# sinamalakouti/CDDMSL

Hardware: AMD Instinct MI355X
Metric: images/sec (train step) VOC+Clipart RN50-C4 (higher is better)
Workload: dtype bf16

## Files before the change

### cddmsl_amd/csrc/gemm_conv.hip

```cpp
#include "common.h"
#include <cstdlib>
#include <type_traits>

namespace {

constexpr int BM = 128, BN = 128, KCH = 8;

struct FastDiv {
  unsigned mul, shr, d;
};
static inline FastDiv make_fastdiv(unsigned d) {
  FastDiv f;
  f.d = d;
  unsigned s = 0;
  while ((1ull << s) < d) ++s;
  f.shr = s;
  f.mul = (unsigned)(((1ull << 32) * ((1ull << s) - d)) / d + 1);
  return f;
}
__device__ __forceinline__ unsigned fdiv(unsigned n, const FastDiv& f) { return (__umulhi(n, f.mul) + n) >> f.shr; }

template <typename T> __device__ __forceinline__ float affine(float v, float sc, float bi) {
  return sizeof(T) <= 2 ? __builtin_fmaf(v, sc, bi) : v * sc + bi;
}
// ... 1821 lines not shown
      continue;
    }
    const unsigned vy = (unsigned)(((tile * 32 + 4 * hh) * p.ldy + r) * ES), vmk = (unsigned)(((tile * 32 + 4 * hh) * p.ldm + r) * ES);
#pragma unroll
    for (int nt = 0; nt < NT; ++nt)
#pragma unroll
      for (int g = 0; g < 16; ++g) {
        const int row = (g & 3) + 8 * (g >> 2);
        float v = affine<T>(acc[nt][g], sc[nt], bi[nt]);
        asm("v_max_f32 %0, %1, %2" : "=v"(v) : "v"(v), "s"(relu_floor));
        if (p.relu_mask) {
          float mv;
          if (ES == 2) mv = bf2f((unsigned)__builtin_amdgcn_raw_buffer_load_b16(rm, vmk, (row * p.ldm + nt * 32) * ES, 0));
          else mv = __builtin_bit_cast(float, __builtin_amdgcn_raw_buffer_load_b32(rm, vmk, (row * p.ldm + nt * 32) * ES, 0));
          if (!(mv > 0.f)) v = 0.f;
        }
        if (ES == 2) __builtin_amdgcn_raw_buffer_store_b16((unsigned short)f2bf(v), ry, vy, (row * p.ldy + nt * 32) * ES, 0);
        else __builtin_amdgcn_raw_buffer_store_b32(__builtin_bit_cast(unsigned, v), ry, vy, (row * p.ldy + nt * 32) * ES, 0);
      }
  }
}

static thread_local int g_last_kernel = 0;
static thread_local int g_plan_only = 0;
static thread_local int g_batch = 1;
static inline int g_batch_peek() { return g_batch; }

__device__ __forceinline__ void blds16(__amdgpu_buffer_rsrc_t r, unsigned voff, unsigned soff, void* l) {
  __builtin_amdgcn_raw_ptr_buffer_load_lds(r, (__attribute__((address_space(3))) void*)l, 16, (int)voff, (int)soff, 0, 0);
}

template <typename T, bool RPOOL, int EPI, bool PRE = false>
__device__ __forceinline__ void tile_epilogue(const ConvArgs& p, f32x16 (&acc)[4][2], float* ep, int wr, int wc, int lane, int m0, int n0,
                                              const u32x4 (*pre)[4] = nullptr, const f32x4* sb = nullptr) {
  constexpr int ES = Mma<T>::ES;
  const int r32 = lane & 31, hh = lane >> 5;
  const int cg = lane & 7, rr = lane >> 3;
  const int n = n0 + wc * 64 + cg * 8;
  float sc[8], bi[8];
#pragma unroll
  for (int j = 0; j < 8; ++j) {
    if (sb) { sc[j] = sb[j >> 2][j & 3]; bi[j] = sb[2 + (j >> 2)][j & 3]; }
    else { sc[j] = p.scale ? p.scale[n + j] : 1.f; bi[j] = p.bias ? p.bias[n + j] : 0.f; }
  }
  const bool has_res = EPI < 0 ? p.residual != nullptr : (EPI & 1) != 0;
  const bool has_msk = EPI < 0 ? p.relu_mask != nullptr : (EPI & 2) != 0;
  const bool f32out = EPI < 0 && (ES == 4 || p.out_f32 != 0);
  const int eso = f32out ? 4 : 2;
  const float relu_floor = p.relu ? 0.f : -__builtin_inff();
  const long rows = p.M - m0;
  auto mk = [&](const char* base, long ld, int es) {
    long bytes = rows * ld * es;
    if (bytes > 0x7fffffffL) bytes = 0x7fffffffL;
    return __builtin_amdgcn_make_buffer_rsrc((void*)(base + (long)m0 * ld * es), 0, base ? (int)bytes : 0, 0x00020000);
  };
// ... 31 lines not shown
        else if (has_res && !rf32) rres_[i][q] = __builtin_amdgcn_raw_buffer_load_b128(rres, vr, (a * 32 + 8 * i) * p.ldr * ES + q * 16, CDDMSL_LOAD_AUX);
        if (has_msk) rmsk_[i][q] = __builtin_amdgcn_raw_buffer_load_b128(rmsk, vm, (a * 32 + 8 * i) * p.ldm * ES + q * 16, CDDMSL_LOAD_AUX);
      }
  };
  if (PRE && DEPTH == 2) {
#pragma unroll
    for (int d = 0; d < 2; ++d)
#pragma unroll
      for (int i = 0; i < 4; ++i) {
        if (EPI & 1) {
          rresb[d % DEPTH][i][0] = pre[d][i];
          if (EPI & 2) rmskb[d % DEPTH][i][0] = __builtin_amdgcn_raw_buffer_load_b128(rmsk, vm, (d * 32 + 8 * i) * p.ldm * ES, CDDMSL_LOAD_AUX);
        } else rmskb[d % DEPTH][i][0] = pre[d][i];
      }
  } else if (DEPTH == 2 && !rf32) { fetch(0, rresb[0], rmskb[0]); fetch(1, rresb[DEPTH - 1], rmskb[DEPTH - 1]); }
  auto put = [&](auto A) {
    constexpr int a = decltype(A)::value;
#pragma unroll
    for (int b = 0; b < 2; ++b)
#pragma unroll
      for (int g = 0; g < 16; ++g)
        *(float*)(wbase[(b << 2) ^ (g & 3)] + ((g & 3) + 8 * (g >> 2)) * 256 + (a & 1) * 8192) = acc[a][b][g];
  };
  auto pass = [&](auto A) {
    constexpr int a = decltype(A)::value;
    if (DEPTH == 1) fetch(a, rresb[0], rmskb[0]);
    if (rf32) {
#pragma unroll
      for (int f = 0; f < 8; ++f)
        rresb[(f >> 2) % DEPTH][f & 3][0] = __builtin_amdgcn_raw_buffer_load_b128(rres, vr, (a * 32 + 8 * (f >> 1)) * p.ldr * 4 + (f & 1) * 16, 0);
    }
    u32x4 (*rres_)[ES / 2] = rresb[a % DEPTH];
    u32x4 (*rmsk_)[ES / 2] = rmskb[a % DEPTH];
    asm volatile("s_waitcnt lgkmcnt(0)" ::: "memory");
    f32x4 val[4][2];
#pragma unroll
    for (int i = 0; i < 4; ++i) {
      const int row = rr + 8 * i;
      const f32x4* src = (const f32x4*)(ep + (a & 1) * 2048 + row * 64 + ((cg ^ (row & 7)) << 3));
      val[i][0] = src[0]; val[i][1] = src[1];
    }
    asm volatile("" ::: "memory");
    if constexpr (a + 1 < 4) put(std::integral_constant<int, a + 1>{});
    asm volatile("" ::: "memory");
#pragma unroll
    for (int i = 0; i < 4; ++i) {
      const f32x4 v0 = val[i][0], v1 = val[i][1];
      float v[8] = {v0[0], v0[1], v0[2], v0[3], v1[0], v1[1], v1[2], v1[3]};
#pragma unroll
      for (int j = 0; j < 8; ++j) v[j] = affine<T>(v[j], sc[j], bi[j]);
      if (rf32) {
#pragma unroll
        for (int j = 0; j < 4; ++j) {
          v[j] += __builtin_bit_cast(f32x4, rresb[((2 * i) >> 2) % DEPTH][(2 * i) & 3][0])[j];
          v[4 + j] += __builtin_bit_cast(f32x4, rresb[((2 * i + 1) >> 2) % DEPTH][(2 * i + 1) & 3][0])[j];
        }
      } else if (RPOOL) {
        if (ES == 2) {
#pragma unroll
          for (int j = 0; j < 4; ++j) { v[2 * j] += 0.25f * bf2f(rres_[i][0][j] & 0xffff); v[2 * j + 1] += 0.25f * bf2f(rres_[i][0][j] >> 16); }
        } else {
#pragma unroll
          for (int j = 0; j < 4; ++j) {
            v[j] += 0.25f * __builtin_bit_cast(f32x4, rres_[i][0])[j]; v[4 + j] += 0.25f * __builtin_bit_cast(f32x4, rres_[i][ES / 2 - 1])[j];
          }
        }
      } else if (has_res) {
        if (ES == 2) {
#pragma unroll
// ... 19 lines not shown
          }
        }
#pragma unroll
        for (int j = 0; j < 8; ++j) if (!(mv[j] > 0.f)) v[j] = 0.f;
      }
      const unsigned so = (unsigned)((a * 32 + 8 * i) * p.ldy * eso);
      if (emit8) {
#pragma unroll
        for (int j = 0; j < 8; ++j) am8 = absmax_bits(am8, v[j]);
        const u32x2 o8 = {pack4_e4m3(v[0] * q8s, v[1] * q8s, v[2] * q8s, v[3] * q8s), pack4_e4m3(v[4] * q8s, v[5] * q8s, v[6] * q8s, v[7] * q8s)};
        __builtin_amdgcn_raw_buffer_store_b64(o8, ry8, vy8, (unsigned)((a * 32 + 8 * i) * p.ldy), CDDMSL_STORE_AUX);
        asm volatile("s_nop 4" ::: "memory");
        asm volatile("" :: "v"(o8));
      }
      if (f32out) {
        const u32x4 o0 = {__builtin_bit_cast(unsigned, v[0]), __builtin_bit_cast(unsigned, v[1]), __builtin_bit_cast(unsigned, v[2]), __builtin_bit_cast(unsigned, v[3])};
        const u32x4 o1 = {__builtin_bit_cast(unsigned, v[4]), __builtin_bit_cast(unsigned, v[5]), __builtin_bit_cast(unsigned, v[6]), __builtin_bit_cast(unsigned, v[7])};
        __builtin_amdgcn_raw_buffer_store_b128(o0, ry, vy, so, CDDMSL_STORE_AUX);
        __builtin_amdgcn_raw_buffer_store_b128(o1, ry, vy, so + 16, CDDMSL_STORE_AUX);
        asm volatile("s_nop 4" ::: "memory");
        asm volatile("" :: "v"(o0), "v"(o1));
      } else {
        const u32x4 o = {pack2bf(v[0], v[1]), pack2bf(v[2], v[3]), pack2bf(v[4], v[5]), pack2bf(v[6], v[7])};
        if (p.nt_out) __builtin_amdgcn_raw_buffer_store_b128(o, ry, vy, so, CDDMSL_STORE_AUX);
        else __builtin_amdgcn_raw_buffer_store_b128(o, ry, vy, so, 0);
        asm volatile("s_nop 4" ::: "memory");
        asm volatile("" :: "v"(o));
      }
    }
    if (DEPTH == 2 && a + 2 < 4 && !rf32) fetch(a + 2, rresb[a % DEPTH], rmskb[a % DEPTH]);
  };
  put(std::integral_constant<int, 0>{});
  pass(std::integral_constant<int, 0>{});
  pass(std::integral_constant<int, 1>{});
  pass(std::integral_constant<int, 2>{});
  pass(std::integral_constant<int, 3>{});
  if (emit8 && p.amax8) {
    am8 = wave_max_u(am8);
    if (lane == 0) atomicMax(p.amax8 + (blockIdx.x & 63), am8);
  }
}

template <typename T, bool TAPS, bool RPOOL = false, int EPI = -1, bool PERSIST = false, bool SPLITK = false>
__global__ __launch_bounds__(512) void k_conv_fwd256(ConvArgs p) {
  __shared__ __attribute__((aligned(16))) u32x4 lds[2 * 2 * 2 * 128 * KCH];
  const int t_in = threadIdx.x;
  p.x += (long)blockIdx.y * p.bx; p.w += (long)blockIdx.y * p.bw; p.y += (long)blockIdx.y * p.by;
  const int ntn = p.Cout >> 8;
  const int ntiles = PERSIST ? (p.tile_limit ? p.tile_limit : ntn * ((p.M + 255) >> 8)) : 0;
  int lbid = PERSIST ? (int)((blockIdx.x & 7) * (gridDim.x >> 3) + (blockIdx.x >> 3))
           : SPLITK ? p.tile0 + (int)(blockIdx.x / (unsigned)p.ksplits) : xcd_remap(blockIdx.x, gridDim.x);
  const int kt0 = SPLITK ? (int)(blockIdx.x % (unsigned)p.ksplits) * p.kper : 0;
  if (PERSIST && lbid >= ntiles) return;
  for (;;) {
  int t = t_in;
  if (PERSIST) asm volatile("" : "+v"(t));
  const int lane = t & 63;
#ifdef CDDMSL_TILE_STAMPS
  const unsigned long long ts_entry = __builtin_amdgcn_s_memrealtime();
#endif
  const int wvu = __builtin_amdgcn_readfirstlane(t >> 6);
  const int wr = wvu >> 2, wc = wvu & 3;
  const int tile_n = lbid % ntn, tile_m = lbid / ntn;
  const int m0 = tile_m * 256, n0 = tile_n * 256;
  const int cl = (t & 7) ^ ((t >> 4) & 7);
  const int nkt = SPLITK ? min(p.kper, (p.Kc >> 3) - kt0) : (p.Kc >> 3);
  const int tpt = p.cpp >> 3;

  auto rowoff = [&](int m, int& iy0, int& ix0) {
    const unsigned tq = fdiv((unsigned)m, p.dWo), ox = m - tq * p.Wo;
    const unsigned img = fdiv(tq, p.dHo), oy = tq - img * p.Ho;
    iy0 = (int)oy * p.stride - p.pad; ix0 = (int)ox * p.stride - p.pad;
    return (((long)img * p.Hi + iy0) * p.Wi + ix0) * p.xrs * 16;
  };
  int iyb, ixb;
  const long base_a = rowoff(m0, iyb, ixb);
  const __amdgpu_buffer_rsrc_t ra_rsrc = __builtin_amdgcn_make_buffer_rsrc((void*)(p.x + base_a), 0, 0x7fffffff, 0x00020000);
  const __amdgpu_buffer_rsrc_t rb_rsrc = __builtin_amdgcn_make_buffer_rsrc((void*)(p.w + (long)n0 * p.wrs * 16), 0, 0x7fffffff, 0x00020000);
  unsigned va[2][2], vinv[2][2], vb[2][2];
  int iy0[2][2], ix0[2][2];
#pragma unroll
  for (int h = 0; h < 2; ++h)
#pragma unroll
    for (int i = 0; i < 2; ++i) {
      const int m = m0 + i * 128 + h * 64 + (t >> 3);
      const bool vm = m < p.M;
      const long ro = rowoff(vm ? m : m0, iy0[h][i], ix0[h][i]);
      va[h][i] = (unsigned)(ro - base_a) + cl * 16;
      if (!vm) { iy0[h][i] = -(1 << 20); if (!TAPS) va[h][i] |= 0x80000000u; }
      vinv[h][i] = 0;
      vb[h][i] = (unsigned)(((2 * i + (t >> 8)) * 64 + h * 32 + ((t >> 3) & 31)) * p.wrs + cl) * 16;
    }
  if (TAPS) {
    unsigned xm[2][2] = {{0, 0}, {0, 0}};
    for (int kx = 0; kx < p.KW; ++kx)
#pragma unroll
      for (int h = 0; h < 2; ++h)
#pragma unroll
        for (int i = 0; i < 2; ++i) xm[h][i] |= ((unsigned)(ix0[h][i] + kx) >= (unsigned)p.Wi ? 1u : 0u) << kx;
    const unsigned full = (1u << p.KW) - 1u;
    for (int ky = 0; ky < p.KH; ++ky)
#pragma unroll
      for (int h = 0; h < 2; ++h)
#pragma unroll
        for (int i = 0; i < 2; ++i) vinv[h][i] |= ((unsigned)(iy0[h][i] + ky) >= (unsigned)p.Hi ? full : xm[h][i]) << (ky * p.KW);
  }
  const int step_col = (p.xrs - (p.cpp - KCH)) * 16;
  const int step_row = ((p.Wi - (p.KW - 1)) * p.xrs - (p.cpp - KCH)) * 16;
  int left[2] = {tpt, tpt}, tap[2] = {0, 0}, kxs[2] = {0, 0};
  unsigned soa[2] = {0, 0}, sob[2] = {0, 0};
  if (SPLITK) {
    const int tap0 = TAPS ? kt0 / tpt : 0, within = TAPS ? kt0 - tap0 * tpt : kt0;
    const int ky0 = TAPS ? tap0 / p.KW : 0, kx0 = tap0 - ky0 * p.KW;
#pragma unroll
    for (int h = 0; h < 2; ++h) {
      left[h] = tpt - (TAPS ? within : 0); tap[h] = tap0; kxs[h] = kx0;
      soa[h] = (unsigned)((ky0 * p.Wi + kx0) * p.xrs * 16 + within * KCH * 16);
      sob[h] = (unsigned)(kt0 * KCH * 16);
    }
  }

  char* const L = (char*)lds;
  auto stageA = [&](auto H, int buf) {
    constexpr int h = decltype(H)::value;
    char* dst = L + (buf << 16) + (h << 14) + wvu * 1024;
#pragma unroll
    for (int i = 0; i < 2; ++i) {
      unsigned v = va[h][i];
      if (TAPS) v |= __builtin_amdgcn_ubfe(vinv[h][i], (unsigned)tap[h], 1u) << 31;
      blds16(ra_rsrc, v, soa[h], dst + i * 8192);
    }
    if (TAPS) {
      int step = KCH * 16;
      if (--left[h] == 0) {
        left[h] = tpt; ++tap[h];
        if (++kxs[h] == p.KW) { kxs[h] = 0; step = step_row; } else step = step_col;
      }
      soa[h] += step;
    } else soa[h] += KCH * 16;
  };
  auto stageB = [&](auto J, int buf) {
    constexpr int j = decltype(J)::value;
    char* dst = L + (buf << 16) + (1 << 15) + (j << 14) + wvu * 1024;
#pragma unroll
    for (int i = 0; i < 2; ++i) blds16(rb_rsrc, vb[j][i], sob[j], dst + i * 8192);
    sob[j] += KCH * 16;
  };
  using I0 = std::integral_constant<int, 0>;
  using I1 = std::integral_constant<int, 1>;

  f32x16 acc[4][2];
#pragma unroll
  for (int a = 0; a < 4; ++a)
#pragma unroll
    for (int b = 0; b < 2; ++b)
#pragma unroll
      for (int r = 0; r < 16; ++r) acc[a][b][r] = 0.f;

  const int r32 = lane & 31, hh = lane >> 5, sw = (r32 >> 1) & 7;
  unsigned ada[4], adb[4];
#pragma unroll
  for (int ks = 0; ks < 4; ++ks) {
    ada[ks] = (unsigned)(((wr * 64 + r32) * KCH + ((2 * ks + hh) ^ sw)) * 16);
    adb[ks] = (unsigned)(((wc * 32 + r32) * KCH + ((2 * ks + hh) ^ sw)) * 16 + (1 << 15));
  }
  u32x4 fa0[2][4], fa1[2][4], fb0[4], fb1[4];
  auto readA = [&](auto I, u32x4 (*fa)[4]) {
    constexpr int i = decltype(I)::value;
// ... 20 lines not shown
  unsigned long long st_sum[4] = {0, 0, 0, 0}, st_last = 0;
#define CDDMSL_STAMP(K) { asm volatile("s_waitcnt lgkmcnt(0)" ::: "memory"); unsigned long long tt_ = __builtin_readcyclecounter(); \
                          asm volatile("s_waitcnt lgkmcnt(0)" ::: "memory"); st_sum[K] += tt_ - st_last; st_last = tt_; }
#else
#define CDDMSL_STAMP(K)
#endif
#define CDDMSL_PHASE_SYNC_IN()                                                      \
  CDDMSL_STAMP(0)                                                                   \
  __builtin_amdgcn_sched_barrier(0);                                                \
  __builtin_amdgcn_s_barrier();                                                     \
  asm volatile("s_waitcnt lgkmcnt(0)" ::: "memory");                                \
  CDDMSL_STAMP(1)                                                                   \
  __builtin_amdgcn_sched_barrier(0);                                                \
  __builtin_amdgcn_s_setprio(1);
#define CDDMSL_PHASE_SYNC_OUT(I, J)                                                 \
  asm volatile("" : "+v"(acc[2 * (I)][J]), "+v"(acc[2 * (I) + 1][J]));    \
  __builtin_amdgcn_s_setprio(0);                                                    \
  CDDMSL_STAMP(2)                                                                   \
  __builtin_amdgcn_sched_barrier(0);                                                \
  __builtin_amdgcn_s_barrier();                                                     \
  CDDMSL_STAMP(3)                                                                   \
  __builtin_amdgcn_sched_barrier(0);

  stageA(I0{}, 0); stageA(I1{}, 0); stageB(I0{}, 0); stageB(I1{}, 0);
  if (nkt > 1) {
    stageA(I0{}, 1); stageB(I0{}, 1); stageB(I1{}, 1);
    asm volatile("s_waitcnt vmcnt(6)" ::: "memory");
  } else {
    asm volatile("s_waitcnt vmcnt(0)" ::: "memory");
  }
  __builtin_amdgcn_s_barrier();
  readA(I0{}, fa0);
  if (wr == 1) __builtin_amdgcn_s_barrier();
  __builtin_amdgcn_sched_barrier(0);
#ifdef CDDMSL_STAMPS
  st_last = __builtin_readcyclecounter();
#endif
#ifdef CDDMSL_TILE_STAMPS
  const unsigned long long ts_loop = __builtin_amdgcn_s_memrealtime();
#endif

  constexpr bool PREF = EPI > 0 && !RPOOL && Mma<T>::ES == 2 && !SPLITK;
  u32x4 pre[2][4];
  f32x4 sb[4];
  auto ktile = [&](int kt, auto LAST) {
    constexpr bool last = decltype(LAST)::value;
    const int d = kt & 1;
    const bool more1 = !last, more2 = !last && kt + 2 < nkt;
    readB(I0{}, fb0);
    if (more1) stageA(I1{}, d ^ 1);
    CDDMSL_PHASE_SYNC_IN();
    CDDMSL_MMA_QUAD(0, 0, fa0, fb0);
    CDDMSL_PHASE_SYNC_OUT(0, 0);
    readB(I1{}, fb1);
    flipB();
    if (more2) stageA(I0{}, d);
    CDDMSL_PHASE_SYNC_IN();
    CDDMSL_MMA_QUAD(0, 1, fa0, fb1);
    CDDMSL_PHASE_SYNC_OUT(0, 1);
    readA(I1{}, fa1);
    flipA();
    if (more2) {
      stageB(I0{}, d);
      asm volatile("s_waitcnt vmcnt(4)" ::: "memory");
    } else if (more1) {
      asm volatile("s_waitcnt vmcnt(0)" ::: "memory");
    } else if (PREF) {
      const bool is_res = (EPI & 1) != 0;
      const char* base = is_res ? p.residual : p.relu_mask;
      const int ld = is_res ? p.ldr : p.ldm;
      long bytes = ((long)p.M - m0) * ld * 2;
      if (bytes > 0x7fffffffL) bytes = 0x7fffffffL;
      const __amdgpu_buffer_rsrc_t rs = __builtin_amdgcn_make_buffer_rsrc((void*)(base + (long)m0 * ld * 2), 0, (int)bytes, 0x00020000);
      const unsigned vo = (unsigned)(((wr * 128 + (lane >> 3)) * ld + n0 + wc * 64 + (lane & 7) * 8) * 2);
#pragma unroll
      for (int a = 0; a < 2; ++a)
#pragma unroll
        for (int i = 0; i < 4; ++i) pre[a][i] = __builtin_amdgcn_raw_buffer_load_b128(rs, vo, (a * 32 + 8 * i) * ld * 2, 0);
    }
    CDDMSL_PHASE_SYNC_IN();
    CDDMSL_MMA_QUAD(1, 1, fa1, fb1);
    CDDMSL_PHASE_SYNC_OUT(1, 1);
    if (more1) readA(I0{}, fa0);
    if (more2) stageB(I1{}, d);
    if (last && !SPLITK) {
      const int n = n0 + wc * 64 + (lane & 7) * 8;
      const f32x4 one = {1.f, 1.f, 1.f, 1.f}, zero = {0.f, 0.f, 0.f, 0.f};
      sb[0] = p.scale ? *(const f32x4*)(p.scale + n) : one; sb[1] = p.scale ? *(const f32x4*)(p.scale + n + 4) : one;
      sb[2] = p.bias ? *(const f32x4*)(p.bias + n) : zero; sb[3] = p.bias ? *(const f32x4*)(p.bias + n + 4) : zero;
    }
    CDDMSL_PHASE_SYNC_IN();
    CDDMSL_MMA_QUAD(1, 0, fa1, fb0);
    CDDMSL_PHASE_SYNC_OUT(1, 0);
  };
  for (int kt = 0; kt + 1 < nkt; ++kt) ktile(kt, std::false_type{});
  ktile(nkt - 1, std::true_type{});
  if (wr == 0) __builtin_amdgcn_s_barrier();
#ifdef CDDMSL_TILE_STAMPS
  const unsigned long long ts_epi = __builtin_amdgcn_s_memrealtime();
#endif
#ifdef CDDMSL_STAMPS
  if (p.stamps && lane == 0) {
#pragma unroll
    for (int k = 0; k < 4; ++k) p.stamps[((long)blockIdx.x * 8 + wvu) * 4 + k] = st_sum[k];
  }
#endif
#undef CDDMSL_MMA_QUAD
#undef CDDMSL_PHASE_SYNC_IN
#undef CDDMSL_PHASE_SYNC_OUT
#undef CDDMSL_STAMP

  if (SPLITK) {
    f32x4* dst = (f32x4*)p.partial + (long)blockIdx.x * (8 * 32 * 64) + (wvu * 32) * 64 + lane;
#pragma unroll
    for (int a = 0; a < 4; ++a)
#pragma unroll
      for (int b = 0; b < 2; ++b)
#pragma unroll
        for (int g4 = 0; g4 < 4; ++g4) {
          const f32x4 v = {acc[a][b][4 * g4], acc[a][b][4 * g4 + 1], acc[a][b][4 * g4 + 2], acc[a][b][4 * g4 + 3]};
          dst[((a * 2 + b) * 4 + g4) * 64] = v;
        }
    return;
  }
  tile_epilogue<T, RPOOL, EPI, PREF>(p, acc, (float*)lds + wvu * 4096, wr, wc, lane, m0, n0, pre, sb);
#ifdef CDDMSL_TILE_STAMPS
  if (p.tstamps && lane == 0) {
    if (!PERSIST) asm volatile("s_waitcnt vmcnt(0)" ::: "memory");
    unsigned long long* o = p.tstamps + ((long)(PERSIST ? lbid : (int)blockIdx.x) * 8 + wvu) * 4;
    o[0] = ts_entry; o[1] = ts_loop; o[2] = ts_epi; o[3] = __builtin_amdgcn_s_memrealtime();
  }
#endif
  if (!PERSIST) break;
  lbid += gridDim.x;
  if (lbid >= ntiles) break;
  __builtin_amdgcn_s_barrier();
  }
}

template <typename T, bool TAPS, int EPI>
__global__ __launch_bounds__(256, 2) void k_conv_fwd2(ConvArgs p) {
  constexpr int SA = 256 * 64, SB = 128 * 64, SS = SA + SB, STAGES = 3;
  __shared__ __attribute__((aligned(16))) u32x4 lds[STAGES * SS / 16];
  const int t = threadIdx.x, lane = t & 63;
#ifdef CDDMSL_TILE_STAMPS
  const unsigned long long ts_entry = __builtin_amdgcn_s_memrealtime();
#endif
  p.x += (long)blockIdx.y * p.bx; p.w += (long)blockIdx.y * p.bw; p.y += (long)blockIdx.y * p.by;
  const int wvu = __builtin_amdgcn_readfirstlane(t >> 6);
  const int wr = wvu >> 1, wc = wvu & 1;
  const int ntn = p.Cout >> 7;
  const int lbid = xcd_remap(blockIdx.x, gridDim.x);
  const int tile_n = lbid % ntn, tile_m = lbid / ntn;
  const int m0 = tile_m * 256, n0 = tile_n * 128;
  const int cl = (t & 3) ^ ((t >> 3) & 3);
  const int nkt = p.Kc >> 2;
  const int tpt = p.cpp >> 2;

  auto rowoff = [&](int m, int& iy0, int& ix0) {
    const unsigned tq = fdiv((unsigned)m, p.dWo), ox = m - tq * p.Wo;
// ... 211 lines not shown
  if (mode == 2) return true;
  if (use_gemm256(a) || g_batch_peek() != 1) return false;
  const char* et = getenv("CDDMSL_FWD2_MIN");
  return (long)(a.Cout / 128) * ((a.M + 255) / 256) >= (et ? atol(et) : 256);
}
template <typename T> void launch_fwd2(const ConvArgs& a, dim3 grid, hipStream_t st) {
  const bool taps = !(a.KH == 1 && a.KW == 1 && a.pad == 0);
  if (sizeof(T) == 4 || a.out_f32 || a.res_f32 || a.y8) {
    if (taps) hipLaunchKernelGGL((k_conv_fwd2<T, true, -1>), grid, dim3(256), 0, st, a);
    else hipLaunchKernelGGL((k_conv_fwd2<T, false, -1>), grid, dim3(256), 0, st, a);
    return;
  }
  if constexpr (sizeof(T) == 2) {
    const int epi = (a.residual ? 1 : 0) | (a.relu_mask ? 2 : 0);
#define CDDMSL_L2(TP, E) hipLaunchKernelGGL((k_conv_fwd2<T, TP, E>), grid, dim3(256), 0, st, a)
    if (taps) { switch (epi) { case 0: CDDMSL_L2(true, 0); break; case 1: CDDMSL_L2(true, 1); break; case 2: CDDMSL_L2(true, 2); break; default: CDDMSL_L2(true, 3); } }
    else { switch (epi) { case 0: CDDMSL_L2(false, 0); break; case 1: CDDMSL_L2(false, 1); break; case 2: CDDMSL_L2(false, 2); break; default: CDDMSL_L2(false, 3); } }
#undef CDDMSL_L2
  }
}

template <typename T, bool TAPS> void launch256_main(const ConvArgs& a, dim3 grid, hipStream_t st, int epi);
constexpr int TAIL_FRAC_DEFAULT = 8;
template <typename T, bool TAPS> void launch256(const ConvArgs& a, dim3 grid, hipStream_t st) {
  if (sizeof(T) == 4 || a.out_f32 || a.res_f32 || a.y8) { hipLaunchKernelGGL((k_conv_fwd256<T, TAPS, false, -1>), grid, dim3(512), 0, st, a); return; }
  const int epi = (a.residual ? 1 : 0) | (a.relu_mask ? 2 : 0);
  if constexpr (std::is_same<T, __bf16>::value) {
    const int ncu = persistent_blocks_raw();
    const int tiles = (int)grid.x, rem = ncu > 0 ? tiles % ncu : 0, nktot = a.Kc >> 3;
    const char* et = getenv("CDDMSL_TAIL_SPLIT");
    const char* ef = getenv("CDDMSL_TAIL_FRAC");
    const int frac = ef ? (atoi(ef) > 0 ? atoi(ef) : 8) : TAIL_FRAC_DEFAULT;
    if (!(et && atoi(et) == 0) && grid.y == 1 && tiles > ncu && rem > 0 && rem * frac <= ncu && nktot >= 16 && g_ws) {
      int S = ncu / rem;
      if (S > nktot / 2) S = nktot / 2;
      { const char* es = getenv("CDDMSL_TAIL_MAXS"); if (es && S > atoi(es)) S = atoi(es); }
      const int kper = (nktot + S - 1) / S;
      S = (nktot + kper - 1) / kper;
      if (S >= 2 && (long)rem * S * 65536 * 4 <= g_ws_bytes) {
        ConvArgs m = a, t = a;
        m.tile_limit = tiles - rem;
        launch256_main<T, TAPS>(m, dim3((unsigned)(tiles - rem), 1), st, epi);
        t.partial = (float*)g_ws; t.tile0 = tiles - rem; t.ksplits = S; t.kper = kper;
        hipLaunchKernelGGL((k_conv_fwd256<T, TAPS, false, -1, false, true>), dim3((unsigned)(rem * S)), dim3(512), 0, st, t);
        hipLaunchKernelGGL(k_conv_split_reduce, dim3((unsigned)(rem * 64)), dim3(256), 0, st, t);
        return;
      }
    }
  }
  launch256_main<T, TAPS>(a, grid, st, epi);
}
template <typename T, bool TAPS> void launch256_main(const ConvArgs& a, dim3 grid, hipStream_t st, int epi) {
  if constexpr (std::is_same<T, __bf16>::value && !TAPS) {
    const int nb = persistent_blocks();
    const char* emk = getenv("CDDMSL_PERSIST_MAXKT");
    if (nb > 0 && grid.y == 1 && (int)grid.x > nb && (a.Kc >> 3) <= (emk ? atoi(emk) : 8)) {
      switch (epi) {
        case 0: hipLaunchKernelGGL((k_conv_fwd256<T, false, false, 0, true>), dim3(nb), dim3(512), 0, st, a); break;
        case 1: hipLaunchKernelGGL((k_conv_fwd256<T, false, false, 1, true>), dim3(nb), dim3(512), 0, st, a); break;
        case 2: hipLaunchKernelGGL((k_conv_fwd256<T, false, false, 2, true>), dim3(nb), dim3(512), 0, st, a); break;
        default: hipLaunchKernelGGL((k_conv_fwd256<T, false, false, 3, true>), dim3(nb), dim3(512), 0, st, a); break;
      }
      return;
    }
  }
  switch (epi) {
    case 0: hipLaunchKernelGGL((k_conv_fwd256<T, TAPS, false, 0>), grid, dim3(512), 0, st, a); break;
    case 1: hipLaunchKernelGGL((k_conv_fwd256<T, TAPS, false, 1>), grid, dim3(512), 0, st, a); break;
    case 2: hipLaunchKernelGGL((k_conv_fwd256<T, TAPS, false, 2>), grid, dim3(512), 0, st, a); break;
    default: hipLaunchKernelGGL((k_conv_fwd256<T, TAPS, false, 3>), grid, dim3(512), 0, st, a); break;
  }
}
template <> void launch256<float, false>(const ConvArgs& a, dim3 grid, hipStream_t st) { hipLaunchKernelGGL((k_conv_fwd256<float, false, false, -1>), grid, dim3(512), 0, st, a); }
template <> void launch256<float, true>(const ConvArgs& a, dim3 grid, hipStream_t st) { hipLaunchKernelGGL((k_conv_fwd256<float, true, false, -1>), grid, dim3(512), 0, st, a); }

template <typename T> int conv_fwd_launch(ConvArgs& a, hipStream_t st) {
  int ntn = (a.Cout + BN - 1) / BN, ntm = (a.M + BM - 1) / BM;
  long grid = (long)ntn * ntm;
  if (grid <= 0) return CDDMSL_OK;
  if (grid > 0x7fffffffL) return CDDMSL_ERR_ARG;
  if (!a.pool && a.KH == 3 && a.KW == 3 && a.pad == 1 && (a.cpp == 1 || a.cpp == 4 || (a.cpp == 8 && a.Cout == 64)) &&
      (a.Cout == 32 || a.Cout == 64) && !a.residual && !a.out_f32 && g_batch == 1 && a.xrs == a.cpp && a.wrs == a.Kc) {
    g_last_kernel = 8;
    if (g_plan_only) return CDDMSL_OK;
    const int nb = a.cpp > 1 ? 256 * 2 : 256 * 8;
    if (a.cpp == 1 && a.Cout == 32) hipLaunchKernelGGL((k_conv3x3_small<T, 1, 1>), dim3(nb), dim3(256), 0, st, a);
    else if (a.cpp == 1) hipLaunchKernelGGL((k_conv3x3_small<T, 1, 2>), dim3(nb), dim3(256), 0, st, a);
    else if (a.cpp == 8) hipLaunchKernelGGL((k_conv3x3_small<T, 8, 2>), dim3(nb), dim3(256), 0, st, a);
// ... 17 lines not shown
    launch_fwd2<T>(a, dim3((unsigned)grid, (unsigned)g_batch), st);
    return launch_status();
  }
  if (use_gemm256(a)) {
    grid = (long)(a.Cout / 256) * ((a.M + 255) / 256);
    g_last_kernel = 3;
    if (g_plan_only) return CDDMSL_OK;
    const dim3 g256((unsigned)grid, (unsigned)g_batch);
    if (a.res_pool) hipLaunchKernelGGL((k_conv_fwd256<T, false, true>), g256, dim3(512), 0, st, a);
    else if (a.KH == 1 && a.KW == 1 && a.pad == 0) launch256<T, false>(a, g256, st);
    else launch256<T, true>(a, g256, st);
  } else if (a.pool) { g_last_kernel = 2; if (g_plan_only) return CDDMSL_OK; hipLaunchKernelGGL(k_conv_fwd_reg<T>, dim3((unsigned)grid), dim3(256), 0, st, a); }
  else { g_last_kernel = 1; if (g_plan_only) return CDDMSL_OK; hipLaunchKernelGGL(k_conv_fwd<T>, dim3((unsigned)grid, (unsigned)g_batch), dim3(256), 0, st, a); }
  return launch_status();
}

}

#ifdef CDDMSL_TILE_STAMPS
static unsigned long long* g_tile_stamps = nullptr;
extern "C" void cddmsl_debug_tile_stamps(unsigned long long* p) { g_tile_stamps = p; }
#endif
extern "C" int cddmsl_last_kernel(void) { return g_last_kernel; }
extern "C" int cddmsl_plan_only(int on) { const int was = g_plan_only; g_plan_only = on; return was; }

static int nt_out_for(long out_bytes) {
  static const long nt_min_mb = getenv("CDDMSL_NT_MIN_MB") ? atol(getenv("CDDMSL_NT_MIN_MB")) : 128;
  return out_bytes > (nt_min_mb << 20) ? 1 : 0;
}

static int conv_fwd_impl(const void* x, const void* w, void* y, const float* scale, const float* bias,
                         const void* residual, const void* relu_mask, int Nimg, int Hi, int Wi, int Cin,
                         int Cout, int KH, int KW, int stride, int pad, int pool, int ldy, int ldr, int ldm,
                         int relu, int out_f32, int dtype, void* y8, const float* q8, float* amax8, void* stream) {
  int es = dtype == 0 ? 2 : 4;
  if (dtype != 0 && dtype != 1) return CDDMSL_ERR_ARG;
  if (Nimg < 0 || Hi <= 0 || Wi <= 0 || Cin <= 0 || Cout <= 0 || KH <= 0 || KW <= 0 || stride <= 0) return CDDMSL_ERR_ARG;
  if ((Cin * es) % 16 != 0) return CDDMSL_ERR_ARG;
  if (pool && (KH != 1 || KW != 1 || pad != 0 || stride != 1)) return CDDMSL_ERR_ARG;
  ConvArgs a;
  a.x = (const char*)x; a.w = (const char*)w; a.y = (char*)y; a.scale = scale; a.bias = bias;
  a.residual = (const char*)residual; a.relu_mask = (const char*)relu_mask;
  a.Nimg = Nimg; a.Hi = Hi; a.Wi = Wi; a.Cin = Cin; a.Cout = Cout; a.KH = KH; a.KW = KW; a.stride = stride; a.pad = pad;
  if (pool) { a.Ho = Hi / 2; a.Wo = Wi / 2; }
  else { a.Ho = (Hi + 2 * pad - KH) / stride + 1; a.Wo = (Wi + 2 * pad - KW) / stride + 1; }
  if (a.Ho <= 0 || a.Wo <= 0) return CDDMSL_ERR_ARG;
// ... 404 lines not shown
```

### include/cddmsl_hip.h

```cpp
#ifndef CDDMSL_HIP_H
#define CDDMSL_HIP_H
#include <stddef.h>

#ifdef __cplusplus
extern "C" {
#endif

int cddmsl_abi_version(void);

int cddmsl_conv_fwd(const void* x, const void* w, void* y, const float* scale, const float* bias, const void* residual,
                    const void* relu_mask, int Nimg, int Hi, int Wi, int Cin, int Cout, int KH, int KW, int stride, int pad,
                    int pool, int ldy, int ldr, int ldm, int relu, int out_f32, int dtype, void* stream);
int cddmsl_set_workspace(void* ptr, long bytes);
int cddmsl_conv_wgrad(const void* x, const void* dy, float* dw, const float* scale, int Nimg, int Hi, int Wi, int Cin,
                      int Cout, int KH, int KW, int stride, int pad, int pool, int ldd, int dtype, void* stream);
int cddmsl_gemm_nt_batched(const void* a, const void* w, void* c, const float* bias, int M, int N, int K, int lda, int ldb, int ldc,
                           int batch, long sa, long sw, long sc, int out_f32, int dtype, void* stream);
int cddmsl_gemm_tn_batched(const void* a, const void* b, void* out, int M, int N, int K, int lda, int ldb, int ldo, int batch, long sa,
                           long sb, long so, int mode, int dtype, void* stream);
int cddmsl_last_kernel(void);
int cddmsl_plan_only(int on);
int cddmsl_weight_prep(const float* w, const float* scale, void* w_fwd, void* w_dgrad, int Cout, int KH, int KW, int Cin,
                       int dtype, void* stream);
int cddmsl_weight_prep_multi(const long long* table, int count, int dtype, void* stream);

int cddmsl_quantize_fp8(const void* x, void* y, const float* scale, float* amax, long numel, int src_dtype, void* stream);
int cddmsl_conv_fwd_fp8(const void* x, const void* w, void* y, const float* scale, const float* bias, const void* residual,
                        const void* relu_mask, int Nimg, int Hi, int Wi, int Cin, int Cout, int KH, int KW, int pad, int relu,
                        int out_f32, void* y8, const float* q8, float* amax8, void* stream);
int cddmsl_conv_fwd_q8(const void* x, const void* w, void* y, const float* scale, const float* bias, const void* residual,
                       const void* relu_mask, int Nimg, int Hi, int Wi, int Cin, int Cout, int KH, int KW, int stride, int pad,
                       int relu, void* y8, const float* q8, float* amax8, void* stream);
int cddmsl_fp8_dot_nt(const void* a, const void* b, float* c, const float* alpha, int R, int N, int K, int ldc, void* stream);
int cddmsl_conv_wgrad_fp8_ok(int Cin, int Cout, int KH, int KW, int pad, int ldd);
int cddmsl_conv_wgrad_fp8(const void* x8, const void* dy8, float* dw, const float* scale, int Nimg, int Hi, int Wi, int Cin, int Cout,
                          int KH, int KW, int pad, int ldd, void* stream);

int cddmsl_roi_align_forward(const void* x, const float* rois, void* y, void* y_pooled, int* dbg_grid, int N, int C, int H, int W,
                             int K, int ph, int pw, float spatial_scale, int sampling_ratio, int aligned, int dtype, void* stream);
int cddmsl_roi_align_backward(const void* dy, const float* rois, const int* roi_start, void* dx, float* ws_ay, float* ws_ax,
                              int* ws_fp, int N, int C, int H, int W, int K, int ph, int pw, float spatial_scale,
                              int sampling_ratio, int aligned, int dtype, void* stream);
int cddmsl_roi_align_forward_affine(const void* x, const float* rois, void* y, void* y_pooled, const float* scale,
// ... 125 lines not shown
```

Measured before the change: 160.2.

## Prefetch next persistent tile's operands during epilogue in 1x1 bf16 conv

Adds a carried variant of the persistent 256-tile 1x1 bf16 forward conv. It issues the next tile's first two K-stage global-to-LDS loads before running the current tile's epilogue, so operand fetch overlaps the epilogue and the barrier between tiles is dropped. The epilogue moves to a separate LDS region written in 16-register halves, and the vmcnt waits are retuned to account for the in-flight carried loads. The variant is chosen by a heuristic based on K-tiles, epilogue type and tile count, and can be overridden with an env var. It costs extra LDS, more register pressure and more intricate wait counting.

```diff
diff --git a/cddmsl_amd/csrc/gemm_conv.hip b/cddmsl_amd/csrc/gemm_conv.hip
--- a/cddmsl_amd/csrc/gemm_conv.hip
+++ b/cddmsl_amd/csrc/gemm_conv.hip
@@ -1867,6 +1867,7 @@
 }
 
 static thread_local int g_last_kernel = 0;
+static thread_local int g_last_form256 = 0;
 static thread_local int g_plan_only = 0;
 static thread_local int g_batch = 1;
 static inline int g_batch_peek() { return g_batch; }
@@ -1875,7 +1876,7 @@
   __builtin_amdgcn_raw_ptr_buffer_load_lds(r, (__attribute__((address_space(3))) void*)l, 16, (int)voff, (int)soff, 0, 0);
 }
 
-template <typename T, bool RPOOL, int EPI, bool PRE = false>
+template <typename T, bool RPOOL, int EPI, bool PRE = false, bool CARRY = false, int NT = -1>
 __device__ __forceinline__ void tile_epilogue(const ConvArgs& p, f32x16 (&acc)[4][2], float* ep, int wr, int wc, int lane, int m0, int n0,
                                               const u32x4 (*pre)[4] = nullptr, const f32x4* sb = nullptr) {
   constexpr int ES = Mma<T>::ES;
@@ -1953,6 +1954,14 @@
       for (int g = 0; g < 16; ++g)
         *(float*)(wbase[(b << 2) ^ (g & 3)] + ((g & 3) + 8 * (g >> 2)) * 256 + (a & 1) * 8192) = acc[a][b][g];
   };
+  auto put16 = [&](auto A, auto S) {
+    constexpr int a = decltype(A)::value, s = decltype(S)::value;
+#pragma unroll
+    for (int b = 0; b < 2; ++b)
+#pragma unroll
+      for (int g = 8 * s; g < 8 * s + 8; ++g)
+        *(float*)(wbase[(b << 2) ^ (g & 3)] + ((g & 3) + 8 * ((g >> 2) & 1)) * 256) = acc[a][b][g];
+  };
   auto pass = [&](auto A) {
     constexpr int a = decltype(A)::value;
     if (DEPTH == 1) fetch(a, rresb[0], rmskb[0]);
@@ -1963,8 +1972,9 @@
     }
     u32x4 (*rres_)[ES / 2] = rresb[a % DEPTH];
     u32x4 (*rmsk_)[ES / 2] = rmskb[a % DEPTH];
+    f32x4 val[4][2];
+    if constexpr (!CARRY) {
     asm volatile("s_waitcnt lgkmcnt(0)" ::: "memory");
-    f32x4 val[4][2];
 #pragma unroll
     for (int i = 0; i < 4; ++i) {
       const int row = rr + 8 * i;
@@ -1974,8 +1984,24 @@
     asm volatile("" ::: "memory");
     if constexpr (a + 1 < 4) put(std::integral_constant<int, a + 1>{});
     asm volatile("" ::: "memory");
+    }
 #pragma unroll
     for (int i = 0; i < 4; ++i) {
+      if constexpr (CARRY) {
+        if ((i & 1) == 0) {
+          asm volatile("s_waitcnt lgkmcnt(0)" ::: "memory");
+#pragma unroll
+          for (int k = 0; k < 2; ++k) {
+            const int row = rr + 8 * k;
+            const f32x4* src = (const f32x4*)(ep + row * 64 + ((cg ^ (row & 7)) << 3));
+            val[i + k][0] = src[0]; val[i + k][1] = src[1];
+          }
+          asm volatile("" ::: "memory");
+          if (i == 0) put16(A, std::integral_constant<int, 1>{});
+          else if constexpr (a + 1 < 4) put16(std::integral_constant<int, a + 1>{}, std::integral_constant<int, 0>{});
+          asm volatile("" ::: "memory");
+        }
+      }
       const f32x4 v0 = val[i][0], v1 = val[i][1];
       float v[8] = {v0[0], v0[1], v0[2], v0[3], v1[0], v1[1], v1[2], v1[3]};
 #pragma unroll
@@ -2041,7 +2067,7 @@
         asm volatile("" :: "v"(o0), "v"(o1));
       } else {
         const u32x4 o = {pack2bf(v[0], v[1]), pack2bf(v[2], v[3]), pack2bf(v[4], v[5]), pack2bf(v[6], v[7])};
-        if (p.nt_out) __builtin_amdgcn_raw_buffer_store_b128(o, ry, vy, so, CDDMSL_STORE_AUX);
+        if (NT < 0 ? p.nt_out != 0 : NT != 0) __builtin_amdgcn_raw_buffer_store_b128(o, ry, vy, so, CDDMSL_STORE_AUX);
         else __builtin_amdgcn_raw_buffer_store_b128(o, ry, vy, so, 0);
         asm volatile("s_nop 4" ::: "memory");
         asm volatile("" :: "v"(o));
@@ -2049,7 +2075,8 @@
     }
     if (DEPTH == 2 && a + 2 < 4 && !rf32) fetch(a + 2, rresb[a % DEPTH], rmskb[a % DEPTH]);
   };
-  put(std::integral_constant<int, 0>{});
+  if constexpr (CARRY) put16(std::integral_constant<int, 0>{}, std::integral_constant<int, 0>{});
+  else put(std::integral_constant<int, 0>{});
   pass(std::integral_constant<int, 0>{});
   pass(std::integral_constant<int, 1>{});
   pass(std::integral_constant<int, 2>{});
@@ -2060,9 +2087,11 @@
   }
 }
 
-template <typename T, bool TAPS, bool RPOOL = false, int EPI = -1, bool PERSIST = false, bool SPLITK = false>
+template <int EPI> constexpr int carry_younger() { return 16 + (EPI ? 8 : 0); }
+template <typename T, bool TAPS, bool RPOOL = false, int EPI = -1, bool PERSIST = false, bool SPLITK = false, bool CARRY = false, int NT = -1>
 __global__ __launch_bounds__(512) void k_conv_fwd256(ConvArgs p) {
-  __shared__ __attribute__((aligned(16))) u32x4 lds[2 * 2 * 2 * 128 * KCH];
+  static_assert(!CARRY || (PERSIST && !TAPS && !RPOOL && !SPLITK && EPI >= 0 && EPI <= 2 && Mma<T>::ES == 2), "carried form: bf16 1x1, one optional epilogue operand");
+  __shared__ __attribute__((aligned(16))) u32x4 lds[2 * 2 * 2 * 128 * KCH + (CARRY ? 8 * 256 : 0)];
   const int t_in = threadIdx.x;
   p.x += (long)blockIdx.y * p.bx; p.w += (long)blockIdx.y * p.bw; p.y += (long)blockIdx.y * p.by;
   const int ntn = p.Cout >> 8;
@@ -2071,8 +2100,16 @@
            : SPLITK ? p.tile0 + (int)(blockIdx.x / (unsigned)p.ksplits) : xcd_remap(blockIdx.x, gridDim.x);
   const int kt0 = SPLITK ? (int)(blockIdx.x % (unsigned)p.ksplits) * p.kper : 0;
   if (PERSIST && lbid >= ntiles) return;
+  int m0, n0;
+  __amdgpu_buffer_rsrc_t ra_rsrc, rb_rsrc;
+  unsigned va[2][2], vinv[2][2], vb[2][2];
+  int left[2], tap[2], kxs[2];
+  unsigned soa[2], sob[2];
+  bool carried = false;
+  const int wv_in = CARRY ? __builtin_amdgcn_readfirstlane(t_in >> 6) : 0;
+  auto thread_index = [&]() { return CARRY ? (wv_in << 6) + (int)__builtin_amdgcn_mbcnt_hi(~0u, __builtin_amdgcn_mbcnt_lo(~0u, 0u)) : t_in; };
   for (;;) {
-  int t = t_in;
+  int t = thread_index();
   if (PERSIST) asm volatile("" : "+v"(t));
   const int lane = t & 63;
 #ifdef CDDMSL_TILE_STAMPS
@@ -2080,9 +2117,6 @@
 #endif
   const int wvu = __builtin_amdgcn_readfirstlane(t >> 6);
   const int wr = wvu >> 2, wc = wvu & 3;
-  const int tile_n = lbid % ntn, tile_m = lbid / ntn;
-  const int m0 = tile_m * 256, n0 = tile_n * 256;
-  const int cl = (t & 7) ^ ((t >> 4) & 7);
   const int nkt = SPLITK ? min(p.kper, (p.Kc >> 3) - kt0) : (p.Kc >> 3);
   const int tpt = p.cpp >> 3;
 
@@ -2092,11 +2126,14 @@
     iy0 = (int)oy * p.stride - p.pad; ix0 = (int)ox * p.stride - p.pad;
     return (((long)img * p.Hi + iy0) * p.Wi + ix0) * p.xrs * 16;
   };
+  auto setup = [&](int lb, int t, bool dead) __attribute__((always_inline)) {
+  const int tile_n = lb % ntn, tile_m = lb / ntn;
+  m0 = tile_m * 256; n0 = tile_n * 256;
+  const int cl = (t & 7) ^ ((t >> 4) & 7);
   int iyb, ixb;
   const long base_a = rowoff(m0, iyb, ixb);
-  const __amdgpu_buffer_rsrc_t ra_rsrc = __builtin_amdgcn_make_buffer_rsrc((void*)(p.x + base_a), 0, 0x7fffffff, 0x00020000);
-  const __amdgpu_buffer_rsrc_t rb_rsrc = __builtin_amdgcn_make_buffer_rsrc((void*)(p.w + (long)n0 * p.wrs * 16), 0, 0x7fffffff, 0x00020000);
-  unsigned va[2][2], vinv[2][2], vb[2][2];
+  ra_rsrc = __builtin_amdgcn_make_buffer_rsrc((void*)(p.x + base_a), 0, 0x7fffffff, 0x00020000);
+  rb_rsrc = __builtin_amdgcn_make_buffer_rsrc((void*)(p.w + (long)n0 * p.wrs * 16), 0, 0x7fffffff, 0x00020000);
   int iy0[2][2], ix0[2][2];
 #pragma unroll
   for (int h = 0; h < 2; ++h)
@@ -2109,6 +2146,7 @@
       if (!vm) { iy0[h][i] = -(1 << 20); if (!TAPS) va[h][i] |= 0x80000000u; }
       vinv[h][i] = 0;
       vb[h][i] = (unsigned)(((2 * i + (t >> 8)) * 64 + h * 32 + ((t >> 3) & 31)) * p.wrs + cl) * 16;
+      if (CARRY && dead) { va[h][i] |= 0x80000000u; vb[h][i] |= 0x80000000u; }
     }
   if (TAPS) {
     unsigned xm[2][2] = {{0, 0}, {0, 0}};
@@ -2124,10 +2162,8 @@
 #pragma unroll
         for (int i = 0; i < 2; ++i) vinv[h][i] |= ((unsigned)(iy0[h][i] + ky) >= (unsigned)p.Hi ? full : xm[h][i]) << (ky * p.KW);
   }
-  const int step_col = (p.xrs - (p.cpp - KCH)) * 16;
-  const int step_row = ((p.Wi - (p.KW - 1)) * p.xrs - (p.cpp - KCH)) * 16;
-  int left[2] = {tpt, tpt}, tap[2] = {0, 0}, kxs[2] = {0, 0};
-  unsigned soa[2] = {0, 0}, sob[2] = {0, 0};
+#pragma unroll
+  for (int h = 0; h < 2; ++h) { left[h] = tpt; tap[h] = 0; kxs[h] = 0; soa[h] = 0; sob[h] = 0; }
   if (SPLITK) {
     const int tap0 = TAPS ? kt0 / tpt : 0, within = TAPS ? kt0 - tap0 * tpt : kt0;
     const int ky0 = TAPS ? tap0 / p.KW : 0, kx0 = tap0 - ky0 * p.KW;
@@ -2138,14 +2174,18 @@
       sob[h] = (unsigned)(kt0 * KCH * 16);
     }
   }
+  };
+  if (!CARRY || !carried) setup(lbid, t, false);
+  const int step_col = (p.xrs - (p.cpp - KCH)) * 16;
+  const int step_row = ((p.Wi - (p.KW - 1)) * p.xrs - (p.cpp - KCH)) * 16;
 
   char* const L = (char*)lds;
-  auto stageA = [&](auto H, int buf) {
+  auto stageA = [&](auto H, int buf, unsigned kill = 0u) {
     constexpr int h = decltype(H)::value;
     char* dst = L + (buf << 16) + (h << 14) + wvu * 1024;
 #pragma unroll
     for (int i = 0; i < 2; ++i) {
-      unsigned v = va[h][i];
+      unsigned v = va[h][i] | kill;
       if (TAPS) v |= __builtin_amdgcn_ubfe(vinv[h][i], (unsigned)tap[h], 1u) << 31;
       blds16(ra_rsrc, v, soa[h], dst + i * 8192);
     }
@@ -2158,11 +2198,11 @@
       soa[h] += step;
     } else soa[h] += KCH * 16;
   };
-  auto stageB = [&](auto J, int buf) {
+  auto stageB = [&](auto J, int buf, unsigned kill = 0u) {
     constexpr int j = decltype(J)::value;
     char* dst = L + (buf << 16) + (1 << 15) + (j << 14) + wvu * 1024;
 #pragma unroll
-    for (int i = 0; i < 2; ++i) blds16(rb_rsrc, vb[j][i], sob[j], dst + i * 8192);
+    for (int i = 0; i < 2; ++i) blds16(rb_rsrc, vb[j][i] | kill, sob[j], dst + i * 8192);
     sob[j] += KCH * 16;
   };
   using I0 = std::integral_constant<int, 0>;
@@ -2229,12 +2269,21 @@
   CDDMSL_STAMP(3)                                                                   \
   __builtin_amdgcn_sched_barrier(0);
 
-  stageA(I0{}, 0); stageA(I1{}, 0); stageB(I0{}, 0); stageB(I1{}, 0);
-  if (nkt > 1) {
-    stageA(I0{}, 1); stageB(I0{}, 1); stageB(I1{}, 1);
-    asm volatile("s_waitcnt vmcnt(6)" ::: "memory");
+  if (CARRY && carried) {
+    wait_vm<8 + carry_younger<EPI>()>();
+  } else if (CARRY) {
+    const unsigned k1 = (unsigned)(nkt - 2) & 0x80000000u;
+    stageA(I0{}, 0); stageA(I1{}, 0); stageB(I0{}, 0); stageB(I1{}, 0);
+    stageA(I0{}, 1, k1); stageA(I1{}, 1, k1); stageB(I0{}, 1, k1); stageB(I1{}, 1, k1);
+    wait_vm<8>();
   } else {
-    asm volatile("s_waitcnt vmcnt(0)" ::: "memory");
+    stageA(I0{}, 0); stageA(I1{}, 0); stageB(I0{}, 0); stageB(I1{}, 0);
+    if (nkt > 1) {
+      stageA(I0{}, 1); stageB(I0{}, 1); stageB(I1{}, 1);
+      asm volatile("s_waitcnt vmcnt(6)" ::: "memory");
+    } else {
+      asm volatile("s_waitcnt vmcnt(0)" ::: "memory");
+    }
   }
   __builtin_amdgcn_s_barrier();
   readA(I0{}, fa0);
@@ -2250,12 +2299,12 @@
   constexpr bool PREF = EPI > 0 && !RPOOL && Mma<T>::ES == 2 && !SPLITK;
   u32x4 pre[2][4];
   f32x4 sb[4];
-  auto ktile = [&](int kt, auto LAST) {
-    constexpr bool last = decltype(LAST)::value;
+  auto ktile = [&](int kt, auto LAST, auto FIRSTC) {
+    constexpr bool last = decltype(LAST)::value, firstc = decltype(FIRSTC)::value;
     const int d = kt & 1;
     const bool more1 = !last, more2 = !last && kt + 2 < nkt;
     readB(I0{}, fb0);
-    if (more1) stageA(I1{}, d ^ 1);
+    if (more1 && !firstc) stageA(I1{}, d ^ 1);
     CDDMSL_PHASE_SYNC_IN();
     CDDMSL_MMA_QUAD(0, 0, fa0, fb0);
     CDDMSL_PHASE_SYNC_OUT(0, 0);
@@ -2267,7 +2316,10 @@
     CDDMSL_PHASE_SYNC_OUT(0, 1);
     readA(I1{}, fa1);
     flipA();
-    if (more2) {
+    if (firstc && carried) {
+      if (more2) { stageB(I0{}, d); wait_vm<4 + carry_younger<EPI < 0 ? 0 : EPI>()>(); }
+      else wait_vm<carry_younger<EPI < 0 ? 0 : EPI>()>();
+    } else if (more2) {
       stageB(I0{}, d);
       asm volatile("s_waitcnt vmcnt(4)" ::: "memory");
     } else if (more1) {
@@ -2300,8 +2352,13 @@
     CDDMSL_MMA_QUAD(1, 0, fa1, fb0);
     CDDMSL_PHASE_SYNC_OUT(1, 0);
   };
-  for (int kt = 0; kt + 1 < nkt; ++kt) ktile(kt, std::false_type{});
-  ktile(nkt - 1, std::true_type{});
+  if constexpr (CARRY) {
+    if (nkt > 1) ktile(0, std::false_type{}, std::true_type{});
+    for (int kt = 1; kt + 1 < nkt; ++kt) ktile(kt, std::false_type{}, std::false_type{});
+  } else {
+    for (int kt = 0; kt + 1 < nkt; ++kt) ktile(kt, std::false_type{}, std::false_type{});
+  }
+  ktile(nkt - 1, std::true_type{}, std::false_type{});
   if (wr == 0) __builtin_amdgcn_s_barrier();
 #ifdef CDDMSL_TILE_STAMPS
   const unsigned long long ts_epi = __builtin_amdgcn_s_memrealtime();
@@ -2330,7 +2387,18 @@
         }
     return;
   }
-  tile_epilogue<T, RPOOL, EPI, PREF>(p, acc, (float*)lds + wvu * 4096, wr, wc, lane, m0, n0, pre, sb);
+  const int em0 = m0, en0 = n0;
+  if constexpr (CARRY) {
+    const int nx = lbid + (int)gridDim.x;
+    int t2 = thread_index();
+    asm volatile("" : "+v"(t2));
+    setup(nx, t2, nx >= ntiles);
+    const unsigned k1 = (unsigned)(nkt - 2) & 0x80000000u;
+    stageA(I0{}, 0); stageA(I1{}, 0); stageB(I0{}, 0); stageB(I1{}, 0);
+    stageA(I0{}, 1, k1); stageA(I1{}, 1, k1); stageB(I0{}, 1, k1); stageB(I1{}, 1, k1);
+    carried = true;
+  }
+  tile_epilogue<T, RPOOL, EPI, PREF, CARRY, NT>(p, acc, CARRY ? (float*)lds + 32768 + wvu * 1024 : (float*)lds + wvu * 4096, wr, wc, lane, em0, en0, pre, sb);
 #ifdef CDDMSL_TILE_STAMPS
   if (p.tstamps && lane == 0) {
     if (!PERSIST) asm volatile("s_waitcnt vmcnt(0)" ::: "memory");
@@ -2341,8 +2409,9 @@
   if (!PERSIST) break;
   lbid += gridDim.x;
   if (lbid >= ntiles) break;
-  __builtin_amdgcn_s_barrier();
-  }
+  if (!CARRY) __builtin_amdgcn_s_barrier();
+  }
+  if (CARRY) asm volatile("s_waitcnt vmcnt(0)" ::: "memory");
 }
 
 template <typename T, bool TAPS, int EPI>
@@ -2600,6 +2669,10 @@
 
 template <typename T, bool TAPS> void launch256_main(const ConvArgs& a, dim3 grid, hipStream_t st, int epi);
 constexpr int TAIL_FRAC_DEFAULT = 8;
+static bool carry_rule(int nkt, int epi, int tiles, int nb) {
+  static const unsigned char ok[9] = {0, 0x1, 0x3, 0, 0x7, 0, 0, 0, 0x6};
+  return nkt <= 8 && ((ok[nkt] >> epi) & 1) && tiles >= 3 * nb;
+}
 template <typename T, bool TAPS> void launch256(const ConvArgs& a, dim3 grid, hipStream_t st) {
   if (sizeof(T) == 4 || a.out_f32 || a.res_f32 || a.y8) { hipLaunchKernelGGL((k_conv_fwd256<T, TAPS, false, -1>), grid, dim3(512), 0, st, a); return; }
   const int epi = (a.residual ? 1 : 0) | (a.relu_mask ? 2 : 0);
@@ -2632,7 +2705,24 @@
   if constexpr (std::is_same<T, __bf16>::value && !TAPS) {
     const int nb = persistent_blocks();
     const char* emk = getenv("CDDMSL_PERSIST_MAXKT");
+    const char* ec = getenv("CDDMSL_CARRY");
+    const int cmode = ec ? atoi(ec) : 1;
+    if (nb > 0 && grid.y == 1 && epi <= 2 && (cmode == 2 || (cmode == 1 && carry_rule(a.Kc >> 3, epi, (int)grid.x, nb)))) {
+      g_last_form256 = 2;
+#define CDDMSL_LC(E, N) hipLaunchKernelGGL((k_conv_fwd256<T, false, false, E, true, false, true, N>), dim3(nb), dim3(512), 0, st, a)
+      switch (epi * 2 + (a.nt_out ? 1 : 0)) {
+        case 0: CDDMSL_LC(0, 0); break;
+        case 1: CDDMSL_LC(0, 1); break;
+        case 2: CDDMSL_LC(1, 0); break;
+        case 3: CDDMSL_LC(1, 1); break;
+        case 4: CDDMSL_LC(2, 0); break;
+        default: CDDMSL_LC(2, 1); break;
+      }
+#undef CDDMSL_LC
+      return;
+    }
     if (nb > 0 && grid.y == 1 && (int)grid.x > nb && (a.Kc >> 3) <= (emk ? atoi(emk) : 8)) {
+      g_last_form256 = 1;
       switch (epi) {
         case 0: hipLaunchKernelGGL((k_conv_fwd256<T, false, false, 0, true>), dim3(nb), dim3(512), 0, st, a); break;
         case 1: hipLaunchKernelGGL((k_conv_fwd256<T, false, false, 1, true>), dim3(nb), dim3(512), 0, st, a); break;
@@ -2642,6 +2732,7 @@
       return;
     }
   }
+  g_last_form256 = 0;
   switch (epi) {
     case 0: hipLaunchKernelGGL((k_conv_fwd256<T, TAPS, false, 0>), grid, dim3(512), 0, st, a); break;
     case 1: hipLaunchKernelGGL((k_conv_fwd256<T, TAPS, false, 1>), grid, dim3(512), 0, st, a); break;
@@ -2705,6 +2796,7 @@
 extern "C" void cddmsl_debug_tile_stamps(unsigned long long* p) { g_tile_stamps = p; }
 #endif
 extern "C" int cddmsl_last_kernel(void) { return g_last_kernel; }
+extern "C" int cddmsl_last_fwd256_form(void) { return g_last_form256; }
 extern "C" int cddmsl_plan_only(int on) { const int was = g_plan_only; g_plan_only = on; return was; }
 
 static int nt_out_for(long out_bytes) {
diff --git a/include/cddmsl_hip.h b/include/cddmsl_hip.h
--- a/include/cddmsl_hip.h
+++ b/include/cddmsl_hip.h
@@ -19,6 +19,7 @@
 int cddmsl_gemm_tn_batched(const void* a, const void* b, void* out, int M, int N, int K, int lda, int ldb, int ldo, int batch, long sa,
                            long sb, long so, int mode, int dtype, void* stream);
 int cddmsl_last_kernel(void);
+int cddmsl_last_fwd256_form(void);
 int cddmsl_plan_only(int on);
 int cddmsl_weight_prep(const float* w, const float* scale, void* w_fwd, void* w_dgrad, int Cout, int KH, int KW, int Cin,
                        int dtype, void* stream);
```

New measurement: 162.3, median of 6. 1.3% higher.
